# AjayGaneshC/medical-segmentation-pytorch

Hardware: AMD Instinct MI355X
Metric: images/sec (whole node) + val Dice, DUCKNet-17 352x352 at 1/2/4/8 MI355X (higher is better)
Workload: dtype bf16; 1 GPU; model=DUCKNet-17, global_batch=320, per_gpu_batch=320, seq_len=123904, step=SegTrainer.train_step, image_size=352, parallelism=dp1, impl=fused, optimizer=adam, loss=ce, syncbn=False, hipgraph=True

## Files before the change

csrc/bindings.cpp:

```cpp
#include <torch/extension.h>
#include <c10/hip/HIPStream.h>

#include <algorithm>
#include <vector>

#include "launchers.h"

namespace {

hipStream_t cur_stream() { return c10::hip::getCurrentHIPStream().stream(); }

#define CHECK_DEV(t) TORCH_CHECK((t).is_cuda() && (t).is_contiguous(), #t " must be a contiguous GPU tensor")
#define CHECK_BF16(t) CHECK_DEV(t); TORCH_CHECK((t).scalar_type() == at::kBFloat16, #t " must be bf16")
#define CHECK_F32(t) CHECK_DEV(t); TORCH_CHECK((t).scalar_type() == at::kFloat, #t " must be fp32")
#define CHECK_I64(t) CHECK_DEV(t); TORCH_CHECK((t).scalar_type() == at::kLong, #t " must be int64")

inline uint16_t* bf(const at::Tensor& t) { return reinterpret_cast<uint16_t*>(t.data_ptr()); }
inline float* f32(const at::Tensor& t) { return t.data_ptr<float>(); }
inline const float* f32_opt(const c10::optional<at::Tensor>& t) {
  if (!t.has_value() || !t->defined()) return nullptr;
  CHECK_F32(*t);
  return t->data_ptr<float>();
}
inline float* f32_opt_mut(const c10::optional<at::Tensor>& t) { return const_cast<float*>(f32_opt(t)); }
// ... 1602 lines not shown

extern "C" const char* msp_sources_sha();

PYBIND11_MODULE(_C, m) {
  m.doc() = "MI355X (gfx950) HIP kernels for medical_segmentation_pytorch_amd";
  m.def("conv_fwd", &conv_fwd, py::arg("xs"), py::arg("wp"), py::arg("ys"), py::arg("bias"), py::arg("stat_part"),
        py::arg("dims"), py::arg("dy"), py::arg("dx"), py::arg("trans"), py::arg("xc") = OptTensors{},
        py::arg("xrelu") = 0, py::arg("accumulate") = false, py::arg("gy") = OptTensors{},
        py::arg("gs") = OptTensors{}, py::arg("gk") = OptTensors{}, py::arg("grelu") = 0);
  m.def("conv_fwd_bn", &conv_fwd_bn, py::arg("xs"), py::arg("wp"), py::arg("ys"), py::arg("stat_part"), py::arg("dims"),
        py::arg("dy"), py::arg("dx"), py::arg("bn_y"), py::arg("bn_coef"), py::arg("relu"), py::arg("gy") = OptTensors{},
        py::arg("gs") = OptTensors{}, py::arg("gk") = OptTensors{}, py::arg("grelu") = 0);
  m.def("conv_wgrad", &conv_wgrad_t, py::arg("dys"), py::arg("xs"), py::arg("dw"), py::arg("dims"), py::arg("dy"),
        py::arg("dx"), py::arg("trans"), py::arg("xc") = OptTensors{}, py::arg("xrelu") = 0,
        py::arg("gy") = OptTensors{}, py::arg("gs") = OptTensors{}, py::arg("gk") = OptTensors{}, py::arg("grelu") = 0);
  m.def("conv_wgrad_uses_halo", &conv_wgrad_uses_halo_t);
  m.def("conv_pick_mi", &conv_pick_mi);
  m.def("conv_rows_alloc", &conv_rows_alloc);
  m.def("conv_stat_blocks", &conv_stat_blocks_t, py::arg("dims"), py::arg("dy"), py::arg("dx"), py::arg("trans") = false,
        py::arg("bwd") = false, py::arg("bne") = false);
  m.def("conv_uses_halo", &conv_uses_halo_t, py::arg("dims"), py::arg("dy"), py::arg("dx"), py::arg("trans"),
        py::arg("bwd") = false);
  m.def("conv_set_halo", [](bool on) { conv_set_halo(on ? 1 : 0); });
  m.def("conv_set_halo_split", [](int64_t mode) { conv_set_halo_split((int)mode); });
  m.def("conv_set_gemm", [](bool on) { conv_gemm_set(on ? 1 : 0); });
  m.def("conv_gemm_force_cfg", [](int64_t c) { conv_gemm_force_cfg((int)c); });
  m.def("conv_gemm_num_cfgs", []() { return conv_gemm_num_cfgs(); });
  m.def("conv_gemm_stamp_buffer", [](c10::optional<at::Tensor> buf) {
    if (!buf.has_value()) return conv_gemm_stamp_buffer(nullptr, 0);
    TORCH_CHECK(buf->is_cuda() && buf->is_contiguous() && buf->scalar_type() == at::kLong && buf->dim() == 2 &&
                    buf->size(1) == 4, "conv_gemm_stamp_buffer: a contiguous int64 [blocks][4] device tensor");
    return conv_gemm_stamp_buffer(buf->data_ptr(), buf->size(0));
  });
  m.def("conv_set_wgrad_gemm", [](int64_t mode) { conv_wgrad_gemm_set((int)mode); });
  m.def("conv_wgrad_gemm_force_cfg", [](int64_t c) { conv_wgrad_gemm_force_cfg((int)c); });
  m.def("conv_wgrad_gemm_num_cfgs", []() { return conv_wgrad_gemm_num_cfgs(); });
  m.def("conv_uses_wgrad_gemm", [](std::vector<int64_t> dims, std::vector<int64_t> dy, std::vector<int64_t> dx, bool trans) {
    return conv_wgrad_gemm_ok(make_geom(dims, dy, dx), trans);
  });
  m.def("conv_uses_gemm", [](std::vector<int64_t> dims, std::vector<int64_t> dy, std::vector<int64_t> dx, bool trans) {
    return conv_gemm_ok(make_geom(dims, dy, dx), trans);
  });
  m.def("conv_set_phase", [](bool on) { conv_set_phase(on ? 1 : 0); });
  m.def("pack_weight", &pack_weight_t);
  m.def("unpack_wgrad", &unpack_wgrad_t, py::arg("src"), py::arg("dst"), py::arg("nrow"), py::arg("nch"),
        py::arg("T"), py::arg("Cpk"), py::arg("Ktot"), py::arg("t_base"), py::arg("c_base"), py::arg("s_row"),
        py::arg("s_ch"), py::arg("accumulate"), py::arg("nrep") = 1, py::arg("rep_stride") = 0);
  m.def("conv_wgrad_replicas", &conv_wgrad_replicas_t, py::arg("dims"), py::arg("dy"), py::arg("dx"), py::arg("trans"),
        py::arg("bwd") = false, py::arg("pro") = false);
  m.def("pack_batch", &pack_batch_t);
  m.def("pack_per_block", &pack_per_block);
  m.def("bn_partial_blocks", [](int64_t P, int64_t Cp) { return bn_partial_blocks(P, Cp); });
  m.def("sum_stats", &sum_stats_t, py::arg("inputs"), py::arg("out"), py::arg("part"), py::arg("P"), py::arg("Cp"),
        py::arg("coefs") = OptTensors{}, py::arg("relu_mask") = 0);
  m.def("bn_reduce_partials", &bn_reduce_partials_t);
  m.def("bn_reduce_splits", [](int64_t nblk) { return bn_reduce_splits(nblk); });
  m.def("bn_collapse", &bn_collapse_t);
  m.def("bn_finalize", &bn_finalize_t);
  m.def("bn_reduce_finalize", &bn_reduce_finalize_t);
  m.def("bn_reduce_bwd_finalize", &bn_reduce_bwd_finalize_t);
  m.def("bn_rf_chunks", [](int64_t Cp) { return bn_rf_chunks((int)Cp); });
  m.def("bn_act_apply", &bn_act_apply_t);
  m.def("bn_act_apply_relu6", &bn_act_apply_relu6_t);
  m.def("bn_add_act", &bn_add_act_t);
  m.def("gconv_fwd", &gconv_fwd_t);
  m.def("relu6", &relu6_t);
// ... 158 lines not shown
```

csrc/conv_gemm.hip:

```cpp
#include <algorithm>

#include "common.h"
#include "launchers.h"

namespace {

typedef float f32x16_t __attribute__((ext_vector_type(16)));
typedef __attribute__((address_space(3))) void lds_void_t;

DEVI f32x16_t mfma32(const uint4& a, const uint4& b, f32x16_t c) {
#ifdef GK_KO_MFMA
  c[0] += __uint_as_float(a.x ^ b.y);
  return c;
#else
  return __builtin_amdgcn_mfma_f32_32x32x16_bf16(as_bf16x8(a), as_bf16x8(b), c, 0, 0, 0);
#endif
}

DEVI void st_stream8(uint16_t* p, uint32_t lo, uint32_t hi) {
#ifdef GK_KO_STORE
  if (lo == 0x7fc17fc1u && hi == 0x12345678u) *reinterpret_cast<uint2*>(p) = make_uint2(lo, hi);
#else
  *reinterpret_cast<uint2*>(p) = make_uint2(lo, hi);
#endif
}

__device__ __attribute__((aligned(64))) uint4 g_zero_page[4];

DEVI void glds16(const void* src, uint32_t lds) {
#ifdef GK_KO_DMA
  return;
#endif
  unsigned keep;
  asm volatile("s_mov_b32 %0, m0\n\ts_mov_b32 m0, %2\n\ts_nop 0\n\tglobal_load_lds_dwordx4 %1, off\n\ts_mov_b32 m0, %0"
               : "=&s"(keep) : "v"(src), "s"(lds) : "memory");
}

typedef __attribute__((address_space(3))) uint8_t lds_u8_t;

#ifdef GK_STAMP
DEVI unsigned long long gk_clock() {
  unsigned long long t;
  __builtin_amdgcn_sched_barrier(0);
  asm volatile("s_memrealtime %0\n\ts_waitcnt lgkmcnt(0)" : "=s"(t)::"memory");
  __builtin_amdgcn_sched_barrier(0);
  return t;
}
#endif


struct KPos { int t, gi, cl; };

DEVI KPos kpos_init(int k, int Cgi, int Gi) {
  const int Cip = Gi * Cgi;
  KPos p;
  p.t = k / Cip;
  const int rem = k - p.t * Cip;
  p.gi = rem / Cgi;
  p.cl = rem - p.gi * Cgi;
  return p;
}

DEVI void kpos_advance(KPos& p, int by, int Cgi, int Gi) {
  p.cl += by;
  while (p.cl >= Cgi) {
    p.cl -= Cgi;
    if (++p.gi == Gi) { p.gi = 0; ++p.t; }
  }
}

struct GemmGeom {
  long M, OHW;
  int n_co, nk;
  int ps, py, px, OWp;
  long OHWp, OW, OHWf;
  long apitch;
#ifdef GK_STAMP
  unsigned long long* stamp;
  long stamp_cap;
#endif
};

template <int WM, int WN, int FM, int FN, int NS, int BK>
struct GemmCfg {
  static constexpr int NW = WM * WN, NT = 64 * NW;
  static constexpr int TCO = 32 * WM * FM, TPX = 32 * WN * FN;
  static constexpr int ROWB = BK * 2, SLOTS = BK / 8, RPI = 1024 / ROWB;
  static constexpr int A_BYTES = TCO * ROWB, B_BYTES = TPX * ROWB, STAGE = A_BYTES + B_BYTES;
  static constexpr int A_INS = TCO / RPI / NW, B_INS = TPX / RPI / NW;
  static constexpr int LDS = NS * STAGE;
  static_assert(BK == 64 || BK == 32, "stage width");
  static_assert(TCO % (RPI * NW) == 0 && TPX % (RPI * NW) == 0, "tile rows must split evenly over the waves");
  static_assert(2 * WN * TCO * 4 <= NS * STAGE, "stats scratch must fit in the staging LDS");
  static_assert(NS >= 2 && NS <= 5 && (NS - 2) * (A_INS + B_INS) < 64, "pipeline depth / vmcnt range");
  static_assert(NW % 2 == 0, "one logical k slot per lane across the wave's DMA instructions");
  static DEVI int swz(int row) { return BK == 64 ? ((row >> 1) & 7) : ((row >> 2) & 3); }
};

struct TapGrid {
  int kw, y0, ys, x0, xs;
  int akw, ar0, ars, ac0, acs;
};

template <int WM, int WN, int FM, int FN, int NS, int BK, bool BNE, int OCC = 2>
__global__ __launch_bounds__(64 * WM * WN, OCC) void conv_gemm_kernel(ConvArgs a, GemmGeom gg, TapGrid tg) {
  using C = GemmCfg<WM, WN, FM, FN, NS, BK>;
  constexpr int kRowB = C::ROWB, RPI = C::RPI;
  const ConvGeom& g = a.g;
  extern __shared__ __attribute__((aligned(16))) uint8_t smem[];

  const int tid = threadIdx.x, lane = tid & 63, wave = __builtin_amdgcn_readfirstlane(tid >> 6);
  const uint32_t sbase = (uint32_t)(uintptr_t)(lds_u8_t*)smem;
#ifdef GK_STAMP
  const unsigned long long ts0 = gk_clock();
  unsigned long long ts1 = ts0;
#endif

  const int nwg = gridDim.x, orig = blockIdx.x;
  const int xq = nwg / 8, xr = nwg % 8, xcd = orig % 8;
  const int wgid = (xcd < xr ? xcd * (xq + 1) : xr * (xq + 1) + (xcd - xr) * xq) + orig / 8;
  const int co_t = wgid % gg.n_co;
  const long px_t = wgid / gg.n_co;
  const int co0 = co_t * C::TCO;
  const long px0 = px_t * C::TPX;
  const int rows = g.Go * g.Cgo;
  const int Cgi = g.Cgi, Gi = g.Gi;
  const int IHW = g.IH * g.IW;

  const int ls = (lane % C::SLOTS) ^ C::swz(RPI * wave + lane / C::SLOTS);
  const uint16_t* zero = reinterpret_cast<const uint16_t*>(g_zero_page);
  const uint16_t* a_src[C::A_INS];
#pragma unroll
  for (int j = 0; j < C::A_INS; ++j) {
    const int co = co0 + RPI * (j * C::NW + wave) + lane / C::SLOTS;
    a_src[j] = a.w + (long)(co < rows ? co : 0) * gg.apitch + 8 * ls;
#ifdef GK_KO_AMISS
    a_src[j] = a.w + 8 * ls;
#endif
  }
  long b_pix[C::B_INS];
  uint32_t b_vm[C::B_INS];
#pragma unroll
  for (int j = 0; j < C::B_INS; ++j) {
    const long m = px0 + RPI * (j * C::NW + wave) + lane / C::SLOTS;
    b_pix[j] = 0;
    b_vm[j] = 0u;
    if (m < gg.M) {
      const int n = (int)(m / gg.OHW);
      const int r = (int)(m - (long)n * gg.OHW);
      const int oh = r / g.OW, ow = r - (r / g.OW) * g.OW;
      const int ih0 = oh * g.stride, iw0 = ow * g.stride;
      b_pix[j] = ((long)n * IHW + (long)ih0 * g.IW + iw0) * Cgi;
#ifdef GK_KO_BMISS
      b_pix[j] = ((long)(ih0 % 4) * g.IW + (iw0 % 8)) * Cgi;
#endif
      uint32_t vm = 0u;
      int tr = 0, tc = 0;
      for (int t = 0; t < g.T; ++t) {
        const int ih = ih0 + tg.y0 + tr * tg.ys, iw = iw0 + tg.x0 + tc * tg.xs;
        if ((unsigned)ih < (unsigned)g.IH && (unsigned)iw < (unsigned)g.IW) vm |= 1u << t;
// ... 12 lines not shown
    g0 = rem / Cgi;
    cl0 = rem - g0 * Cgi;
    tr0 = t0 / tg.kw;
    tc0 = t0 - tr0 * tg.kw;
    toff0 = ((long)(tg.y0 + tr0 * tg.ys) * g.IW + (tg.x0 + tc0 * tg.xs)) * Cgi;
  };
  walk_to(0);
  auto gptr = [&](int q) {
    const uint16_t* xb = a.x[0];
#pragma unroll
    for (int u = 1; u < kMaxGroups; ++u) xb = q == u ? a.x[u] : xb;
    return xb;
  };
  const uint16_t* xg0 = gptr(g0);
  const uint16_t* xg1 = gptr(g0 + 1 == Gi ? 0 : g0 + 1);

  const int Cip_ = Gi * Cgi;
  auto stage = [&](int kt, uint32_t sb) {
    const int kb = kt * BK;
    int g1 = g0 + 1, t1 = t0, tr1 = tr0, tc1 = tc0;
    long toff1 = toff0;
    if (g1 == Gi) {
      g1 = 0;
      ++t1;
      toff1 += dcol;
      if (++tc1 == tg.kw) { tc1 = 0; ++tr1; toff1 += drow; }
    }
    const int rem0 = Cgi - cl0;
    const bool nx = 8 * ls >= rem0;
    const int dA0 = ((tg.ar0 + tr0 * tg.ars) * tg.akw + tg.ac0 + tc0 * tg.acs - t0) * Cip_;
    const int dA1 = t1 < g.T ? ((tg.ar0 + tr1 * tg.ars) * tg.akw + tg.ac0 + tc1 * tg.acs - t1) * Cip_ : dA0;
    const int ka = kb + (nx ? dA1 : dA0);
#pragma unroll
    for (int j = 0; j < C::A_INS; ++j) glds16(a_src[j] + ka, sb + (RPI * (j * C::NW + wave)) * kRowB);
    const int t = nx ? t1 : t0;
#ifdef GK_OLD_XSEL
    const uint16_t* base = (nx ? gptr(g1) : gptr(g0)) + (nx ? toff1 + (8 * ls - rem0) : toff0 + (cl0 + 8 * ls));
#else
    asm volatile("" : "+s"(xg0), "+s"(xg1));
    const uint16_t* base = (nx ? xg1 : xg0) + (nx ? toff1 + (8 * ls - rem0) : toff0 + (cl0 + 8 * ls));
#endif
    const bool tin = t < 32;
#pragma unroll
    for (int j = 0; j < C::B_INS; ++j) {
      const bool ok = tin && ((b_vm[j] >> t) & 1u);
      glds16(ok ? (const void*)(base + b_pix[j]) : (const void*)zero,
             sb + C::A_BYTES + (RPI * (j * C::NW + wave)) * kRowB);
    }
    cl0 += BK;
    if (cl0 >= Cgi) {
      cl0 -= Cgi; g0 = g1; t0 = t1; tr0 = tr1; tc0 = tc1; toff0 = toff1;
      xg0 = xg1;
      xg1 = gptr(g0 + 1 == Gi ? 0 : g0 + 1);
    }
  };

  const int wm = wave / WN, wn = wave - (wave / WN) * WN;
  const int lr = lane & 31, lh = lane >> 5;
  const int key = C::swz(lr);
  constexpr int KS = BK / 16;
  int soff[KS];
#pragma unroll
  for (int s = 0; s < KS; ++s) soff[s] = (((2 * s + lh) ^ key) << 4);
  const int a_row0 = (wm * FM * 32 + lr) * kRowB;
  const int b_row0 = C::A_BYTES + (wn * FN * 32 + lr) * kRowB;

  f32x16_t acc[FM][FN];
#pragma unroll
  for (int i = 0; i < FM; ++i)
#pragma unroll
    for (int j = 0; j < FN; ++j)
#pragma unroll
      for (int e = 0; e < 16; ++e) acc[i][j][e] = 0.f;

  constexpr int INS = C::A_INS + C::B_INS;
  const int nk = gg.nk;
#pragma unroll
  for (int p = 0; p < NS - 1; ++p)
    if (p < nk) stage(p, sbase + p * C::STAGE);
  for (int kt = 0; kt < nk; ++kt) {
    const int ahead = min(nk - 1 - kt, NS - 2);
    if (NS >= 5 && ahead >= 3) asm volatile("s_waitcnt vmcnt(%0)" ::"n"(3 * INS) : "memory");
    else if (NS >= 4 && ahead >= 2) asm volatile("s_waitcnt vmcnt(%0)" ::"n"(2 * INS) : "memory");
    else if (ahead >= 1) asm volatile("s_waitcnt vmcnt(%0)" ::"n"(INS) : "memory");
    else asm volatile("s_waitcnt vmcnt(0)" ::: "memory");
    __builtin_amdgcn_s_barrier();
    __builtin_amdgcn_sched_barrier(0);
    if (kt + NS - 1 < nk) stage(kt + NS - 1, sbase + ((kt + NS - 1) % NS) * C::STAGE);
    const uint8_t* cur = smem + (kt % NS) * C::STAGE;
#ifdef GK_STAMP
    if (kt == 0) ts1 = gk_clock();
#endif
#pragma unroll
    for (int s = 0; s < KS; ++s) {
      uint4 af[FM], bfr[FN];
#pragma unroll
#ifdef GK_KO_LDS
      for (int i = 0; i < FM; ++i) af[i] = make_uint4(kt + i, s, lane, 0);
#pragma unroll
      for (int j = 0; j < FN; ++j) bfr[j] = make_uint4(kt, j + s, 0, lane);
#else
      for (int i = 0; i < FM; ++i) af[i] = *reinterpret_cast<const uint4*>(cur + a_row0 + i * 32 * kRowB + soff[s]);
#pragma unroll
      for (int j = 0; j < FN; ++j) bfr[j] = *reinterpret_cast<const uint4*>(cur + b_row0 + j * 32 * kRowB + soff[s]);
#endif
#pragma unroll
      for (int i = 0; i < FM; ++i)
#pragma unroll
        for (int j = 0; j < FN; ++j) acc[i][j] = mfma32(af[i], bfr[j], acc[i][j]);
    }
  }
  __syncthreads();
#ifdef GK_STAMP
  const unsigned long long ts2 = gk_clock();
#endif

  float* s_st = reinterpret_cast<float*>(smem);
  const bool stats = a.stat_part != nullptr;
#pragma unroll
  for (int i = 0; i < FM; ++i) {
    const int rb = wm * FM * 32 + i * 32;
    uint16_t* yb[4];
    int cl4[4];
    float cs[16], cq[16];
#pragma unroll
    for (int q = 0; q < 4; ++q) {
      const int cb = co0 + rb + 8 * q + 4 * lh;
      const int og = cb < rows ? cb / g.Cgo : 0;
      cl4[q] = cb - og * g.Cgo;
      uint16_t* yg = a.y[0];
#pragma unroll
      for (int t = 1; t < kMaxGroups; ++t) yg = og == t ? a.y[t] : yg;
      yb[q] = cb < rows ? yg + cl4[q] : nullptr;
    }
#pragma unroll
    for (int e = 0; e < 16; ++e) { cs[e] = 0.f; cq[e] = 0.f; }
#pragma unroll
    for (int j = 0; j < FN; ++j) {
      long m = px0 + wn * FN * 32 + j * 32 + lr;
      if (m >= gg.M) continue;
      if (gg.ps) {
        const long n = m / gg.OHWp, r = m - n * gg.OHWp;
        const long oh = r / gg.OWp, ow = r - oh * gg.OWp;
        m = n * gg.OHWf + (gg.py + gg.ps * oh) * gg.OW + gg.px + gg.ps * ow;
      }
#pragma unroll
      for (int q = 0; q < 4; ++q) {
        if (yb[q] == nullptr) continue;
        uint16_t* yp = yb[q] + m * g.Cgo;
        float v[4];
#pragma unroll
        for (int r = 0; r < 4; ++r) v[r] = acc[i][j][4 * q + r];
        if (a.bias != nullptr) {
#pragma unroll
          for (int r = 0; r < 4; ++r) v[r] = cl4[q] + r < g.Cgo_l ? v[r] + a.bias[cl4[q] + r] : 0.f;
        }
        if (!BNE && a.accum) {
          const uint2 ov = *reinterpret_cast<const uint2*>(yp);
          v[0] += __uint_as_float(ov.x << 16); v[1] += __uint_as_float(ov.x & 0xffff0000u);
          v[2] += __uint_as_float(ov.y << 16); v[3] += __uint_as_float(ov.y & 0xffff0000u);
        }
        const uint32_t lo = pack2(v[0], v[1]), hi = pack2(v[2], v[3]);
        st_stream8(yp, lo, hi);
        const float w4[4] = {__uint_as_float(lo << 16), __uint_as_float(lo & 0xffff0000u),
                             __uint_as_float(hi << 16), __uint_as_float(hi & 0xffff0000u)};
        if constexpr (BNE) {
          const int cb = cl4[q];
          const uint2 yy = *reinterpret_cast<const uint2*>(a.bn_y + m * g.Cgo + cb);
          const float4 sc = *reinterpret_cast<const float4*>(a.bn_coef + cb);
          const float4 sh = *reinterpret_cast<const float4*>(a.bn_coef + g.Cgo + cb);
          const float4 mu = *reinterpret_cast<const float4*>(a.bn_coef + 2 * g.Cgo + cb);
          const float y4[4] = {__uint_as_float(yy.x << 16), __uint_as_float(yy.x & 0xffff0000u),
                               __uint_as_float(yy.y << 16), __uint_as_float(yy.y & 0xffff0000u)};
          const float s4[4] = {sc.x, sc.y, sc.z, sc.w}, h4[4] = {sh.x, sh.y, sh.z, sh.w};
          const float m4[4] = {mu.x, mu.y, mu.z, mu.w};
#pragma unroll
          for (int r = 0; r < 4; ++r) {
            const float gr = (!a.bn_relu || fmaf(y4[r], s4[r], h4[r]) > 0.f) ? w4[r] : 0.f;
            cs[4 * q + r] += gr;
            cq[4 * q + r] = fmaf(gr, y4[r] - m4[r], cq[4 * q + r]);
          }
        } else {
#pragma unroll
          for (int r = 0; r < 4; ++r) {
            cs[4 * q + r] += w4[r];
            cq[4 * q + r] = fmaf(w4[r], w4[r], cq[4 * q + r]);
          }
        }
      }
    }
    if (stats) {
#pragma unroll
      for (int e = 0; e < 16; ++e) {
        float s = row16_sum(cs[e]), q = row16_sum(cq[e]);
        s += __shfl_xor(s, 16, 64);
        q += __shfl_xor(q, 16, 64);
        if (lr == 0) {
          const int row = rb + 8 * (e >> 2) + 4 * lh + (e & 3);
          s_st[(wn * 2 + 0) * C::TCO + row] = s;
          s_st[(wn * 2 + 1) * C::TCO + row] = q;
        }
      }
    }
  }
  if (stats) {
    __syncthreads();
    constexpr int HALVES = C::TPX / 128, WPH = WN / HALVES;
    static_assert(C::TPX % 128 == 0 && WN % HALVES == 0, "128-pixel stat rows");
    const long nrow = (gg.M + 127) / 128;
    for (int e = tid; e < HALVES * C::TCO; e += C::NT) {
      const int hb = e / C::TCO, c = e - hb * C::TCO;
      const int co = co0 + c;
      const long srow = px0 / 128 + hb;
      if (co >= rows || srow >= nrow) continue;
      float s = 0.f, q = 0.f;
#pragma unroll
      for (int w = 0; w < WPH; ++w) {
        const int wv = hb * WPH + w;
        s += s_st[(wv * 2 + 0) * C::TCO + c];
        q += s_st[(wv * 2 + 1) * C::TCO + c];
      }
      a.stat_part[(srow * 2 + 0) * rows + co] = s;
      a.stat_part[(srow * 2 + 1) * rows + co] = q;
    }
  }
#ifdef GK_STAMP
  const unsigned long long ts3 = gk_clock();
  if (tid == 0 && gg.stamp != nullptr && wgid < gg.stamp_cap) {
    unsigned long long* sp = gg.stamp + 4 * (long)wgid;
    sp[0] = ts0; sp[1] = ts1; sp[2] = ts2; sp[3] = ts3;
  }
#endif
}

struct CfgId { int wm, wn, fm, fn, ns, bk; };
constexpr CfgId kCfgs[] = {
    {2, 2, 3, 2, 2, 64},
    {2, 2, 2, 2, 2, 64},
    {1, 4, 3, 1, 2, 64},
    {1, 4, 5, 1, 2, 64},
    {2, 2, 1, 2, 2, 64},
    {2, 2, 2, 2, 4, 32},
    {2, 2, 3, 2, 4, 32},
    {2, 2, 4, 2, 3, 32},
    {2, 2, 2, 2, 5, 32},
    {2, 2, 2, 2, 2, 32},
};
constexpr int kNumCfgs = sizeof(kCfgs) / sizeof(kCfgs[0]);
constexpr int kPlannerCfgs = 5;
constexpr int kOccCfg = 9;
constexpr int kGemmTPX = 128;

int g_gemm_mode = -1;
int g_gemm_cfg = -1;

void gemm_env() {
  if (g_gemm_mode < 0) {
    const char* e = getenv("MSP_CONV_GEMM");
    g_gemm_mode = (e == nullptr || e[0] != '0') ? 1 : 0;
  }
}

int gemm_pick_cfg(int rows, int nk64) {
  if (g_gemm_cfg >= 0) return g_gemm_cfg;
  int best = 0;
  double best_cost = 1e30;
  for (int c = 0; c < kPlannerCfgs; ++c) {
    const int tco = 32 * kCfgs[c].wm * kCfgs[c].fm;
    const int tiles = cdiv(rows, tco);
    const double cost = (double)tiles * (tco + 48.0);
    if (cost < best_cost - 1e-9) { best_cost = cost; best = c; }
  }
  const int tb = 32 * kCfgs[best].wm * kCfgs[best].fm, to = 32 * kCfgs[kOccCfg].wm * kCfgs[kOccCfg].fm;
  if (nk64 <= 12 && (double)cdiv(rows, to) * to <= 1.35 * cdiv(rows, tb) * tb) return kOccCfg;
  return best;
}

bool tap_grid(const ConvGeom& g, TapGrid& tg) {
  for (int kw = 1; kw <= g.T; ++kw) {
    if (g.T % kw != 0) continue;
    const int kh = g.T / kw;
    tg.kw = kw; tg.y0 = g.dy[0]; tg.x0 = g.dx[0];
    tg.ys = kh > 1 ? g.dy[kw] - g.dy[0] : 0;
    tg.xs = kw > 1 ? g.dx[1] - g.dx[0] : 0;
    bool ok = true;
    for (int t = 0; t < g.T && ok; ++t)
      ok = g.dy[t] == tg.y0 + (t / kw) * tg.ys && g.dx[t] == tg.x0 + (t % kw) * tg.xs;
    if (ok) return true;
  }
  return false;
}

struct GemmPhase {
  int ps = 0, py = 0, px = 0, OHf = 0, OWf = 0;
  long apitch = 0;
  int akw = 0, ar0 = 0, ars = 1, ac0 = 0, acs = 1;
};

#ifdef GK_STAMP
unsigned long long* g_stamp = nullptr;
long g_stamp_cap = 0;
#endif

template <int WM, int WN, int FM, int FN, int NS, int BK, bool BNE, int OCC = 2>
void launch_gemm(const ConvArgs& a, const GemmPhase& ph, hipStream_t s) {
  using C = GemmCfg<WM, WN, FM, FN, NS, BK>;
  const ConvGeom& g = a.g;
  GemmGeom gg;
  gg.OHW = (long)g.OH * g.OW;
  gg.M = (long)g.N * gg.OHW;
  gg.n_co = cdiv(g.Go * g.Cgo, C::TCO);
  gg.nk = cdiv(g.Kp, BK);
  gg.ps = ph.ps; gg.py = ph.py; gg.px = ph.px; gg.OWp = g.OW;
  gg.OHWp = gg.OHW; gg.OW = ph.OWf; gg.OHWf = (long)ph.OHf * ph.OWf;
  gg.apitch = ph.apitch > 0 ? ph.apitch : g.Kp;
  const long blocks = (long)cdiv(gg.M, C::TPX) * gg.n_co;
#ifdef GK_STAMP
  gg.stamp = g_stamp; gg.stamp_cap = g_stamp_cap;
#endif
  static bool attr = false;
  if (!attr) {
    (void)hipFuncSetAttribute(reinterpret_cast<const void*>(&conv_gemm_kernel<WM, WN, FM, FN, NS, BK, BNE, OCC>),
                              hipFuncAttributeMaxDynamicSharedMemorySize, C::LDS);
    attr = true;
  }
  TapGrid tg;
  (void)tap_grid(g, tg);
  if (ph.akw > 0) {
    tg.akw = ph.akw; tg.ar0 = ph.ar0; tg.ars = ph.ars; tg.ac0 = ph.ac0; tg.acs = ph.acs;
  } else {
    tg.akw = tg.kw; tg.ar0 = 0; tg.ars = 1; tg.ac0 = 0; tg.acs = 1;
  }
  hipLaunchKernelGGL((conv_gemm_kernel<WM, WN, FM, FN, NS, BK, BNE, OCC>), dim3((unsigned)blocks), dim3(C::NT), C::LDS, s, a, gg,
                     tg);
}

template <bool BNE>
int dispatch_gemm(const ConvArgs& a, int cfg, const GemmPhase& ph, hipStream_t s) {
  switch (cfg) {
    case 0: launch_gemm<2, 2, 3, 2, 2, 64, BNE>(a, ph, s); return 0;
    case 1: launch_gemm<2, 2, 2, 2, 2, 64, BNE>(a, ph, s); return 0;
    case 2: launch_gemm<1, 4, 3, 1, 2, 64, BNE>(a, ph, s); return 0;
    case 3: launch_gemm<1, 4, 5, 1, 2, 64, BNE>(a, ph, s); return 0;
    case 4: launch_gemm<2, 2, 1, 2, 2, 64, BNE>(a, ph, s); return 0;
    case 5: launch_gemm<2, 2, 2, 2, 4, 32, BNE>(a, ph, s); return 0;
    case 6: launch_gemm<2, 2, 3, 2, 4, 32, BNE>(a, ph, s); return 0;
    case 7: launch_gemm<2, 2, 4, 2, 3, 32, BNE>(a, ph, s); return 0;
    case 8: launch_gemm<2, 2, 2, 2, 5, 32, BNE>(a, ph, s); return 0;
    case 9: launch_gemm<2, 2, 2, 2, 2, 32, BNE, 4>(a, ph, s); return 0;
  }
  return 1;
}

}

static bool gemm_geom_ok(const ConvGeom& g, int min_c) {
  if (g.Cgi < min_c || g.Cgi % 8 != 0 || g.T > 30) return false;
  TapGrid tg;
  if (!tap_grid(g, tg)) return false;
  const long M = (long)g.N * g.OH * g.OW;
  return M >= 1 && (long)cdiv(M, kGemmTPX) * cdiv(g.Go * g.Cgo, 64) < (1L << 31);
}

bool conv_gemm_ok(const ConvGeom& g, bool trans) {
  gemm_env();
  if (!g_gemm_mode || trans) return false;
  return gemm_geom_ok(g, g.stride > 1 ? 32 : 64);
}

static int gemm_tile_for(const ConvGeom& g) {
  const int cfg = gemm_pick_cfg(g.Go * g.Cgo, cdiv(g.Kp, 64));
  return (g.Cgi < 64 && kCfgs[cfg].bk == 64) ? kOccCfg : cfg;
}

void conv_gemm_set(int on) { gemm_env(); g_gemm_mode = on ? 1 : 0; }
void conv_gemm_force_cfg(int cfg) { gemm_env(); g_gemm_cfg = (cfg >= 0 && cfg < kNumCfgs) ? cfg : -1; }
int conv_gemm_num_cfgs() { return kNumCfgs; }
int conv_gemm_stamp_buffer(void* buf, long cap) {
#ifdef GK_STAMP
  g_stamp = static_cast<unsigned long long*>(buf);
  g_stamp_cap = buf != nullptr ? cap : 0;
  return 1;
#else
  (void)buf; (void)cap;
  return 0;
#endif
}

long conv_gemm_stat_blocks(const ConvGeom& g) { return cdiv((long)g.N * g.OH * g.OW, kGemmTPX); }

int conv_gemm(const ConvArgs& a, hipStream_t s) {
  gemm_env();
  for (int i = 0; i < a.g.Gi; ++i)
    if (a.xc[i] != nullptr) return 2;
  const int cfg = gemm_tile_for(a.g);
  const GemmPhase ph;
  return a.bn_y != nullptr ? dispatch_gemm<true>(a, cfg, ph, s) : dispatch_gemm<false>(a, cfg, ph, s);
}

int conv_gemm_phase(const ConvArgs& a0, const int* tA, int KW, int s_, int py, int px, int OHf, int OWf,
                    hipStream_t s) {
  gemm_env();
  ConvArgs a = a0;
  ConvGeom& g = a.g;
  const long apitch = g.Kp;
  g.Kp = (g.T * g.Gi * g.Cgi + 31) / 32 * 32;
  if (g.T < 1 || !g_gemm_mode || !gemm_geom_ok(g, 32) || a.bn_y != nullptr || a.stat_part != nullptr) return 1;
  for (int i = 0; i < g.Gi; ++i)
    if (a.xc[i] != nullptr || a.gy[i] != nullptr) return 1;
  TapGrid tg;
  if (!tap_grid(g, tg)) return 1;
  GemmPhase ph;
  ph.ps = s_; ph.py = py; ph.px = px; ph.OHf = OHf; ph.OWf = OWf; ph.apitch = apitch;
  const int kh = g.T / tg.kw;
  ph.akw = KW;
  ph.ar0 = tA[0] / KW; ph.ac0 = tA[0] % KW;
  ph.ars = kh > 1 ? tA[tg.kw] / KW - ph.ar0 : 0;
  ph.acs = tg.kw > 1 ? tA[1] % KW - ph.ac0 : 0;
  for (int v = 0; v < g.T; ++v)
    if (tA[v] != (ph.ar0 + (v / tg.kw) * ph.ars) * KW + ph.ac0 + (v % tg.kw) * ph.acs) return 1;
  const int cfg = gemm_tile_for(g);
  return dispatch_gemm<false>(a, cfg, ph, s) == 0 ? 0 : 2;
}
```

csrc/conv_wgrad_gemm.hip:

```cpp
#include <algorithm>

#include "common.h"
#include "launchers.h"

namespace {

typedef float f32x16_t __attribute__((ext_vector_type(16)));
typedef short s16x4_t __attribute__((ext_vector_type(4)));
typedef __attribute__((address_space(3))) uint8_t lds_u8_t;

DEVI f32x16_t mfma32(const uint4& a, const uint4& b, f32x16_t c) {
#ifdef GK_KO_MFMA
  c[0] += __uint_as_float(a.x ^ b.y);
  return c;
#else
  return __builtin_amdgcn_mfma_f32_32x32x16_bf16(as_bf16x8(a), as_bf16x8(b), c, 0, 0, 0);
#endif
}

__device__ __attribute__((aligned(64))) uint4 g_wg_zero_page[4];

DEVI void glds16(const void* src, uint32_t lds) {
#ifdef GK_KO_DMA
  return;
// ... 263 lines not shown
    g_wg_mode = e == nullptr ? 1 : (e[0] == '0' ? 0 : (e[0] == '2' ? 2 : 1));
  }
}

int wg_pick(int rows, int KT, bool pro) {
  if (g_wg_cfg >= 0 && (!pro || wg_pro_ok(kWgCfgs[g_wg_cfg].wn, kWgCfgs[g_wg_cfg].fn))) return g_wg_cfg;
  int best = 0;
  double best_cost = 1e30;
  for (int c = 0; c < kNumWgCfgs; ++c) {
    if (pro && !wg_pro_ok(kWgCfgs[c].wn, kWgCfgs[c].fn)) continue;
    const int tco = 32 * kWgCfgs[c].wm * kWgCfgs[c].fm, tk = 32 * kWgCfgs[c].wn * kWgCfgs[c].fn;
    const double nt = (double)cdiv(rows, tco) * cdiv(KT, tk);
    const double cost = nt * ((double)tco * tk + g_wg_stage_cost * (tco + tk));
    if (cost < best_cost) { best_cost = cost; best = c; }
  }
  return best;
}

bool wg_tap_grid(const ConvGeom& g, WgGeom& w) {
  for (int kw = 1; kw <= g.T; ++kw) {
    if (g.T % kw != 0) continue;
    const int kh = g.T / kw;
    w.kw = kw; w.ty0 = g.dy[0]; w.tx0 = g.dx[0];
    w.tys = kh > 1 ? g.dy[kw] - g.dy[0] : 0;
    w.txs = kw > 1 ? g.dx[1] - g.dx[0] : 0;
    bool ok = true;
    for (int t = 0; t < g.T && ok; ++t) ok = g.dy[t] == w.ty0 + (t / kw) * w.tys && g.dx[t] == w.tx0 + (t % kw) * w.txs;
    if (ok) return true;
  }
  return false;
}

struct WgPlan { int cfg; WgGeom w; long blocks; int nsplit; };

WgPlan wg_plan(const ConvGeom& g, bool pro) {
  WgPlan p{};
  p.cfg = wg_pick(g.Go * g.Cgo, g.T * g.Gi * g.Cgi, pro);
  const WgCfg& c = kWgCfgs[p.cfg];
  WgGeom& w = p.w;
  (void)wg_tap_grid(g, w);
  w.M = (long)g.N * g.OH * g.OW;
  w.KT = g.T * g.Gi * g.Cgi;
  w.n_co = cdiv(g.Go * g.Cgo, 32 * c.wm * c.fm);
  w.n_k = cdiv(w.KT, 32 * c.wn * c.fn);
  w.nstages = (int)((w.M + kBP - 1) / kBP);
  const long ntile = (long)w.n_co * w.n_k;
  const long target = c.wm * c.wn >= 8 ? g_wg_blocks / 2 : g_wg_blocks;
  long ns = std::max(1L, std::min((long)w.nstages, target / std::max(1L, ntile)));
  w.stages_per_split = (int)((w.nstages + ns - 1) / ns);
  ns = (w.nstages + w.stages_per_split - 1) / w.stages_per_split;
  p.nsplit = (int)ns;
  p.blocks = ns * ntile;
  w.d_ohw = make_fastdiv((uint32_t)(g.OH * g.OW));
  w.d_ow = make_fastdiv((uint32_t)g.OW);
  return p;
}

template <int WM, int WN, int FM, int FN>
int launch_wg(const WgradPtrs& P, float* dw, const ConvGeom& g, const WgPlan& p, bool pro, hipStream_t s) {
  constexpr int LDS = 2 * kBP * (32 * WM * FM + 32 * WN * FN) * 2;
  static bool attr[2] = {false, false};
  if (pro) {
    if constexpr (!wg_pro_ok(WN, FN)) {
      return 1;
    } else {
    if (!attr[1]) {
      (void)hipFuncSetAttribute(reinterpret_cast<const void*>(&conv_wgrad_gemm_kernel<WM, WN, FM, FN, true>),
                                hipFuncAttributeMaxDynamicSharedMemorySize, LDS);
      attr[1] = true;
    }
    hipLaunchKernelGGL((conv_wgrad_gemm_kernel<WM, WN, FM, FN, true>), dim3((unsigned)p.blocks), dim3(64 * WM * WN),
                       LDS, s, P, dw, g, p.w);
    return 0;
    }
  }
  if (!attr[0]) {
    (void)hipFuncSetAttribute(reinterpret_cast<const void*>(&conv_wgrad_gemm_kernel<WM, WN, FM, FN, false>),
                              hipFuncAttributeMaxDynamicSharedMemorySize, LDS);
    attr[0] = true;
  }
  hipLaunchKernelGGL((conv_wgrad_gemm_kernel<WM, WN, FM, FN, false>), dim3((unsigned)p.blocks), dim3(64 * WM * WN), LDS,
                     s, P, dw, g, p.w);
  return 0;
}


}

bool conv_wgrad_gemm_ok(const ConvGeom& g, bool trans) {
  wg_env();
  if (!g_wg_mode || trans || g.Cgi % 8 != 0 || g.Cgo % 8 != 0) return false;
  WgGeom w{};
  if (!wg_tap_grid(g, w)) return false;
  const long M = (long)g.N * g.OH * g.OW;
  return M < (1L << 31) - 2 * kBP;
}

int conv_wgrad_gemm_replicas(const ConvGeom& g, bool pro) {
  wg_env();
  return wg_plan(g, pro).nsplit;
}

void conv_wgrad_gemm_set(int mode) { wg_env(); g_wg_mode = mode < 0 ? 0 : (mode > 2 ? 2 : mode); }
int conv_wgrad_gemm_mode() { wg_env(); return g_wg_mode; }
void conv_wgrad_gemm_force_cfg(int cfg) { wg_env(); g_wg_cfg = (cfg >= 0 && cfg < kNumWgCfgs) ? cfg : -1; }
int conv_wgrad_gemm_num_cfgs() { return kNumWgCfgs; }

int conv_wgrad_gemm(const WgradPtrs& P, float* dw, const ConvGeom& g, bool prologue, hipStream_t s) {
  const WgPlan p = wg_plan(g, prologue);
  switch (p.cfg) {
    case 0: return launch_wg<2, 2, 2, 2>(P, dw, g, p, prologue, s);
    case 1: return launch_wg<1, 4, 1, 1>(P, dw, g, p, prologue, s);
    case 2: return launch_wg<2, 2, 1, 2>(P, dw, g, p, prologue, s);
    case 3: return launch_wg<2, 2, 2, 1>(P, dw, g, p, prologue, s);
    case 4: return launch_wg<1, 4, 2, 1>(P, dw, g, p, prologue, s);
    case 5: return launch_wg<2, 2, 4, 1>(P, dw, g, p, prologue, s);
    case 6: return launch_wg<2, 4, 4, 2>(P, dw, g, p, prologue, s);
    case 7: return launch_wg<2, 4, 2, 2>(P, dw, g, p, prologue, s);
    case 8: return launch_wg<4, 2, 2, 2>(P, dw, g, p, prologue, s);
  }
  return 1;
}
```

csrc/launchers.h:

```cpp
#pragma once
#include <hip/hip_runtime.h>
#include <stdint.h>

constexpr int kMaxTaps = 49;

constexpr int kMaxGroups = 8;
struct ConvGeom {
  int N, IH, IW;
  int Gi, Cgi;
  int OH, OW;
  int Go, Cgo, Cgo_l;
  int T, Kp;
  int stride;
  int dy[kMaxTaps], dx[kMaxTaps];
};

struct ConvArgs {
  const uint16_t* x[kMaxGroups];
  uint16_t* y[kMaxGroups];
  const uint16_t* w;
  const float* bias;
  float* stat_part;
  const uint16_t* bn_y;
  const float* bn_coef;
// ... 17 lines not shown
  const float* gs[kMaxGroups];
  const float* gk[kMaxGroups];
  unsigned grelu;
};

bool conv_wgrad_gemm_ok(const ConvGeom& g, bool trans);
int conv_wgrad_gemm_replicas(const ConvGeom& g, bool pro = false);
int conv_wgrad_gemm(const WgradPtrs& P, float* dw, const ConvGeom& g, bool prologue, hipStream_t s);
void conv_wgrad_gemm_set(int mode);
int conv_wgrad_gemm_mode();
void conv_wgrad_gemm_force_cfg(int cfg);
int conv_wgrad_gemm_num_cfgs();

int conv_pick_mi(int rows);
int conv_rows_alloc(int rows);
void conv_set_halo(int on);
void conv_set_halo_split(int mode);
void conv_set_phase(int on);
bool conv_uses_halo(const ConvGeom& g, bool trans, bool bwd = false);
long conv_stat_blocks(const ConvGeom& g, bool trans = false, bool bwd = false, bool bne = false);
bool conv_wgrad_uses_halo(const ConvGeom& g, bool trans);
int conv_igemm(const ConvArgs& a, bool trans, hipStream_t s);
const char* conv_error_string(int rc);

bool conv_gemm_ok(const ConvGeom& g, bool trans);
long conv_gemm_stat_blocks(const ConvGeom& g);
int conv_gemm(const ConvArgs& a, hipStream_t s);
int conv_gemm_phase(const ConvArgs& a, const int* tA, int KW, int s_, int py, int px, int OHf, int OWf,
                    hipStream_t s);
void conv_gemm_set(int on);
void conv_gemm_force_cfg(int cfg);
int conv_gemm_num_cfgs();
int conv_gemm_stamp_buffer(void* buf, long cap);
int conv_plan_selfcheck(int verbose);
int conv_wgrad_replicas(const ConvGeom& g, bool trans, bool bwd = false, bool pro = false);
int conv_wgrad(const uint16_t* const* dy, const uint16_t* const* x, float* dw, const ConvGeom& g, bool trans,
               const float* const* xc, unsigned xrelu, hipStream_t s, const uint16_t* const* gy = nullptr,
               const float* const* gs = nullptr, const float* const* gk = nullptr, unsigned grelu = 0);
void pack_weight(const float* src, uint16_t* dst, int nrow, int nch, int T, int Cpk, int Kp, int t_base,
                 int c_base, long s_row, long s_ch, hipStream_t s);
void pack_batch(const int64_t* jobs, const int* prefix, int njobs, int total_blocks, hipStream_t s);
int pack_per_block();
void unpack_wgrad(const float* src, float* dst, int nrow, int nch, int T, int Cpk, int Ktot, int t_base, int c_base,
                  long s_row, long s_ch, bool accumulate, int nrep, long rep_stride, hipStream_t s);

constexpr int kMaxSumInputs = 8;
constexpr int kTailMax = 6;
constexpr int kTailMaxCp = 512;
long bn_partial_blocks(long P, int Cp);
long bn_tail_blocks(long P, int Cp);
void bn_tail_partial(const uint16_t* dz, const uint16_t* ys, const float* ostats, const float* ocoef, int orelu, int k,
                     const uint16_t* const* y, const float* const* st, unsigned relu, float* part, long P, int Cp,
                     hipStream_t s);
void bn_tail_apply(const uint16_t* dz, const uint16_t* ys, const float* ostats, const float* ocoef, int orelu, int k,
                   const uint16_t* const* y, const float* const* st, const float* const* coef, unsigned relu,
                   uint16_t* const* dy, long P, int Cp, hipStream_t s, uint16_t* g = nullptr);
void sum_stats(const uint16_t* const* inputs, const float* const* coefs, unsigned relu_mask, int k, uint16_t* out,
               float* part, long P, int Cp, hipStream_t s);
int bn_reduce_splits(long nblk);
void bn_reduce_partials(const float* part, long nblk, int width, int col_off, int Cp, double* tmp, hipStream_t s);
void bn_collapse(const double* tmp, int S, int Cp, double* out, hipStream_t s);
void bn_finalize(const double* tmp, int S, int C, int Cp, float count, const float* gamma, const float* beta,
                 float* running_mean, float* running_var, float momentum, float eps, int training,
                 float* scale, float* shift, float* mean, float* invstd, hipStream_t s);
int bn_rf_chunks(int Cp);
void bn_reduce_finalize(const float* part, long nblk, int width, int col_off, int C, int Cp, double* tmp,
// ... 282 lines not shown
```

Measured before the change: 674.0 images/sec.

## Add wide-pixel and non-power-of-two channel tiles to conv GEMM planner

Adds four new forward conv GEMM tile configurations with 160/96/128/192 output-channel and 128/256 pixel tiles. A planner cost model picks them by comparing staged bytes per pixel and wave-quantization round-up against the existing 128-pixel choice. To support channel tiles that do not split evenly across waves, weight DMA is predicated per wave and vmcnt waits become per-wave counts. BN statistics reduction is regrouped for 256-pixel tiles. The goal is less redundant staging of A/B tiles and less tile padding on wide layers, at the cost of more kernel instantiations, more complex waits and a heuristic that may misselect. Also adds plan-logging counters exposed to Python.

```diff
diff --git a/csrc/bindings.cpp b/csrc/bindings.cpp
--- a/csrc/bindings.cpp
+++ b/csrc/bindings.cpp
@@ -1658,6 +1658,13 @@
                     buf->size(1) == 4, "conv_gemm_stamp_buffer: a contiguous int64 [blocks][4] device tensor");
     return conv_gemm_stamp_buffer(buf->data_ptr(), buf->size(0));
   });
+  auto plan_log_list = [](const ConvPlanLog& l) {
+    return std::vector<int64_t>{l.launches, l.blocks, l.staged, l.staged_full, l.cfg, l.tco, l.tpx, l.bk, l.ns, l.nk};
+  };
+  m.def("conv_gemm_plan_log", [plan_log_list](bool reset) { return plan_log_list(conv_gemm_plan_log(reset)); },
+        py::arg("reset") = true);
+  m.def("conv_wgrad_gemm_plan_log",
+        [plan_log_list](bool reset) { return plan_log_list(conv_wgrad_gemm_plan_log(reset)); }, py::arg("reset") = true);
   m.def("conv_set_wgrad_gemm", [](int64_t mode) { conv_wgrad_gemm_set((int)mode); });
   m.def("conv_wgrad_gemm_force_cfg", [](int64_t c) { conv_wgrad_gemm_force_cfg((int)c); });
   m.def("conv_wgrad_gemm_num_cfgs", []() { return conv_wgrad_gemm_num_cfgs(); });
diff --git a/csrc/conv_gemm.hip b/csrc/conv_gemm.hip
--- a/csrc/conv_gemm.hip
+++ b/csrc/conv_gemm.hip
@@ -1,4 +1,5 @@
 #include <algorithm>
+#include <cmath>
 
 #include "common.h"
 #include "launchers.h"
@@ -48,6 +49,19 @@
 }
 #endif
 
+
+template <int N>
+DEVI void wait_vm() { asm volatile("s_waitcnt vmcnt(%0)" ::"n"(N) : "memory"); }
+template <int LVL, int B, int A>
+DEVI void wait_stages(int na) {
+  static_assert(LVL * (A + B) < 64, "vmcnt range");
+  if constexpr (A == 0) {
+    wait_vm<LVL * B>();
+  } else {
+    if (na == A) wait_vm<LVL * (A + B)>();
+    else wait_stages<LVL, B, A - 1>(na);
+  }
+}
 
 struct KPos { int t, gi, cl; };
 
@@ -75,6 +89,7 @@
   int ps, py, px, OWp;
   long OHWp, OW, OHWf;
   long apitch;
+  int sg;
 #ifdef GK_STAMP
   unsigned long long* stamp;
   long stamp_cap;
@@ -87,11 +102,13 @@
   static constexpr int TCO = 32 * WM * FM, TPX = 32 * WN * FN;
   static constexpr int ROWB = BK * 2, SLOTS = BK / 8, RPI = 1024 / ROWB;
   static constexpr int A_BYTES = TCO * ROWB, B_BYTES = TPX * ROWB, STAGE = A_BYTES + B_BYTES;
-  static constexpr int A_INS = TCO / RPI / NW, B_INS = TPX / RPI / NW;
+  static constexpr int A_TOT = TCO / RPI, A_INS = (A_TOT + NW - 1) / NW, B_INS = TPX / RPI / NW;
   static constexpr int LDS = NS * STAGE;
   static_assert(BK == 64 || BK == 32, "stage width");
-  static_assert(TCO % (RPI * NW) == 0 && TPX % (RPI * NW) == 0, "tile rows must split evenly over the waves");
-  static_assert(2 * WN * TCO * 4 <= NS * STAGE, "stats scratch must fit in the staging LDS");
+  static_assert(TCO % RPI == 0 && TPX % (RPI * NW) == 0, "pixel rows must split evenly over the waves");
+  static constexpr int STAT_SLOTS = TPX > 128 ? TPX / 32 : WN;
+  static_assert(2 * STAT_SLOTS * TCO * 4 <= NS * STAGE, "stats scratch must fit in the staging LDS");
+  static_assert(TPX == 128 || (TPX == 256 && FN % 2 == 0), "stat groups of 1 or 2 fragments inside a wave");
   static_assert(NS >= 2 && NS <= 5 && (NS - 2) * (A_INS + B_INS) < 64, "pipeline depth / vmcnt range");
   static_assert(NW % 2 == 0, "one logical k slot per lane across the wave's DMA instructions");
   static DEVI int swz(int row) { return BK == 64 ? ((row >> 1) & 7) : ((row >> 2) & 3); }
@@ -126,6 +143,9 @@
   const int rows = g.Go * g.Cgo;
   const int Cgi = g.Cgi, Gi = g.Gi;
   const int IHW = g.IH * g.IW;
+
+  const int a_real = (min(C::TCO, rows - co0) + RPI - 1) / RPI;
+  const int na = wave < a_real ? (a_real - wave + C::NW - 1) / C::NW : 0;
 
   const int ls = (lane % C::SLOTS) ^ C::swz(RPI * wave + lane / C::SLOTS);
   const uint16_t* zero = reinterpret_cast<const uint16_t*>(g_zero_page);
@@ -204,7 +224,8 @@
     const int dA1 = t1 < g.T ? ((tg.ar0 + tr1 * tg.ars) * tg.akw + tg.ac0 + tc1 * tg.acs - t1) * Cip_ : dA0;
     const int ka = kb + (nx ? dA1 : dA0);
 #pragma unroll
-    for (int j = 0; j < C::A_INS; ++j) glds16(a_src[j] + ka, sb + (RPI * (j * C::NW + wave)) * kRowB);
+    for (int j = 0; j < C::A_INS; ++j)
+      if (j < na) glds16(a_src[j] + ka, sb + (RPI * (j * C::NW + wave)) * kRowB);
     const int t = nx ? t1 : t0;
 #ifdef GK_OLD_XSEL
     const uint16_t* base = (nx ? gptr(g1) : gptr(g0)) + (nx ? toff1 + (8 * ls - rem0) : toff0 + (cl0 + 8 * ls));
@@ -245,17 +266,19 @@
 #pragma unroll
       for (int e = 0; e < 16; ++e) acc[i][j][e] = 0.f;
 
-  constexpr int INS = C::A_INS + C::B_INS;
   const int nk = gg.nk;
 #pragma unroll
   for (int p = 0; p < NS - 1; ++p)
     if (p < nk) stage(p, sbase + p * C::STAGE);
   for (int kt = 0; kt < nk; ++kt) {
     const int ahead = min(nk - 1 - kt, NS - 2);
-    if (NS >= 5 && ahead >= 3) asm volatile("s_waitcnt vmcnt(%0)" ::"n"(3 * INS) : "memory");
-    else if (NS >= 4 && ahead >= 2) asm volatile("s_waitcnt vmcnt(%0)" ::"n"(2 * INS) : "memory");
-    else if (ahead >= 1) asm volatile("s_waitcnt vmcnt(%0)" ::"n"(INS) : "memory");
-    else asm volatile("s_waitcnt vmcnt(0)" ::: "memory");
+    bool waited = false;
+    if constexpr (NS >= 5)
+      if (ahead >= 3) { wait_stages<3, C::B_INS, C::A_INS>(na); waited = true; }
+    if constexpr (NS >= 4)
+      if (!waited && ahead >= 2) { wait_stages<2, C::B_INS, C::A_INS>(na); waited = true; }
+    if (!waited && ahead >= 1) { wait_stages<1, C::B_INS, C::A_INS>(na); waited = true; }
+    if (!waited) wait_vm<0>();
     __builtin_amdgcn_s_barrier();
     __builtin_amdgcn_sched_barrier(0);
     if (kt + NS - 1 < nk) stage(kt + NS - 1, sbase + ((kt + NS - 1) % NS) * C::STAGE);
@@ -289,6 +312,8 @@
 
   float* s_st = reinterpret_cast<float*>(smem);
   const bool stats = a.stat_part != nullptr;
+  constexpr bool WIDE = C::TPX > 128;
+  const int sg = WIDE ? gg.sg : FN;
 #pragma unroll
   for (int i = 0; i < FM; ++i) {
     const int rb = wm * FM * 32 + i * 32;
@@ -305,12 +330,31 @@
       for (int t = 1; t < kMaxGroups; ++t) yg = og == t ? a.y[t] : yg;
       yb[q] = cb < rows ? yg + cl4[q] : nullptr;
     }
+    auto reduce_to = [&](int slot) {
+#pragma unroll
+      for (int e = 0; e < 16; ++e) {
+        float s = row16_sum(cs[e]), q = row16_sum(cq[e]);
+        s += __shfl_xor(s, 16, 64);
+        q += __shfl_xor(q, 16, 64);
+        if (lr == 0) {
+          const int row = rb + 8 * (e >> 2) + 4 * lh + (e & 3);
+          s_st[(slot * 2 + 0) * C::TCO + row] = s;
+          s_st[(slot * 2 + 1) * C::TCO + row] = q;
+        }
+      }
+    };
 #pragma unroll
     for (int e = 0; e < 16; ++e) { cs[e] = 0.f; cq[e] = 0.f; }
 #pragma unroll
     for (int j = 0; j < FN; ++j) {
+      if constexpr (WIDE) {
+        if (j > 0 && j % sg == 0) {
+#pragma unroll
+          for (int e = 0; e < 16; ++e) { cs[e] = 0.f; cq[e] = 0.f; }
+        }
+      }
       long m = px0 + wn * FN * 32 + j * 32 + lr;
-      if (m >= gg.M) continue;
+      if (m < gg.M) {
       if (gg.ps) {
         const long n = m / gg.OHWp, r = m - n * gg.OHWp;
         const long oh = r / gg.OWp, ow = r - oh * gg.OWp;
@@ -360,25 +404,20 @@
           }
         }
       }
-    }
-    if (stats) {
-#pragma unroll
-      for (int e = 0; e < 16; ++e) {
-        float s = row16_sum(cs[e]), q = row16_sum(cq[e]);
-        s += __shfl_xor(s, 16, 64);
-        q += __shfl_xor(q, 16, 64);
-        if (lr == 0) {
-          const int row = rb + 8 * (e >> 2) + 4 * lh + (e & 3);
-          s_st[(wn * 2 + 0) * C::TCO + row] = s;
-          s_st[(wn * 2 + 1) * C::TCO + row] = q;
-        }
       }
+      if constexpr (WIDE) {
+        if (stats && j % sg == sg - 1) reduce_to((wn * FN + j) / sg);
+      }
+    }
+    if constexpr (!WIDE) {
+      if (stats) reduce_to(wn);
     }
   }
   if (stats) {
     __syncthreads();
-    constexpr int HALVES = C::TPX / 128, WPH = WN / HALVES;
-    static_assert(C::TPX % 128 == 0 && WN % HALVES == 0, "128-pixel stat rows");
+    constexpr int HALVES = C::TPX / 128;
+    static_assert(C::TPX % 128 == 0, "128-pixel stat rows");
+    const int WPH = WIDE ? 4 / sg : WN;
     const long nrow = (gg.M + 127) / 128;
     for (int e = tid; e < HALVES * C::TCO; e += C::NT) {
       const int hb = e / C::TCO, c = e - hb * C::TCO;
@@ -386,7 +425,6 @@
       const long srow = px0 / 128 + hb;
       if (co >= rows || srow >= nrow) continue;
       float s = 0.f, q = 0.f;
-#pragma unroll
       for (int w = 0; w < WPH; ++w) {
         const int wv = hb * WPH + w;
         s += s_st[(wv * 2 + 0) * C::TCO + c];
@@ -417,10 +455,18 @@
     {2, 2, 4, 2, 3, 32},
     {2, 2, 2, 2, 5, 32},
     {2, 2, 2, 2, 2, 32},
+    {1, 4, 5, 2, 2, 32},
+    {1, 4, 3, 2, 2, 32},
+    {2, 2, 2, 4, 2, 32},
+    {2, 4, 3, 2, 2, 64},
 };
 constexpr int kNumCfgs = sizeof(kCfgs) / sizeof(kCfgs[0]);
 constexpr int kPlannerCfgs = 5;
 constexpr int kOccCfg = 9;
+constexpr int kWide160 = 10, kWide96 = 11, kWide128 = 12, kWide192 = 13;
+constexpr int kCfgBlocksPerCU[] = {2, 2, 2, 2, 2, 2, 2, 2, 2, 4, 2, 3, 2, 1};
+static_assert(sizeof(kCfgBlocksPerCU) / sizeof(int) == kNumCfgs, "one entry per configuration");
+constexpr int kPlanCUs = 256;
 constexpr int kGemmTPX = 128;
 
 int g_gemm_mode = -1;
@@ -433,8 +479,7 @@
   }
 }
 
-int gemm_pick_cfg(int rows, int nk64) {
-  if (g_gemm_cfg >= 0) return g_gemm_cfg;
+int gemm_pick_cfg128(int rows, int nk64) {
   int best = 0;
   double best_cost = 1e30;
   for (int c = 0; c < kPlannerCfgs; ++c) {
@@ -446,6 +491,38 @@
   const int tb = 32 * kCfgs[best].wm * kCfgs[best].fm, to = 32 * kCfgs[kOccCfg].wm * kCfgs[kOccCfg].fm;
   if (nk64 <= 12 && (double)cdiv(rows, to) * to <= 1.35 * cdiv(rows, tb) * tb) return kOccCfg;
   return best;
+}
+
+double gemm_staged_per_px(int rows, int c) {
+  const int tco = 32 * kCfgs[c].wm * kCfgs[c].fm, tpx = 32 * kCfgs[c].wn * kCfgs[c].fn;
+  return (double)cdiv(rows, tco) * (tco + tpx) / tpx;
+}
+double gemm_rounds(int rows, long M, int c) {
+  const int tco = 32 * kCfgs[c].wm * kCfgs[c].fm, tpx = 32 * kCfgs[c].wn * kCfgs[c].fn;
+  return (double)cdiv(M, (long)tpx) * cdiv(rows, tco) / (kPlanCUs * kCfgBlocksPerCU[c]);
+}
+double gemm_round_up(int rows, long M, int c) {
+  const double x = gemm_rounds(rows, M, c);
+  return x <= 2.0 ? std::ceil(x) / x : 1.0;
+}
+
+int gemm_pick_cfg(int rows, int nk64, int gi, int cgi, long M, bool phase) {
+  if (g_gemm_cfg >= 0) return g_gemm_cfg;
+  const int c128 = gemm_pick_cfg128(rows, nk64);
+  if (gi != 1 || cgi < 64 || phase) return c128;
+  if (c128 == kOccCfg) {
+    const int w = rows <= 96 ? kWide96 : kWide128;
+    const bool ok = nk64 >= 8 && gemm_rounds(rows, M, w) >= 1.0 && gemm_round_up(rows, M, w) <= gemm_round_up(rows, M, c128);
+    return ok ? w : c128;
+  }
+  const double cost128 = gemm_staged_per_px(rows, c128) * gemm_round_up(rows, M, c128);
+  if (gemm_rounds(rows, M, kWide160) >= 1.0 &&
+      gemm_staged_per_px(rows, kWide160) * gemm_round_up(rows, M, kWide160) <= 0.78 * cost128)
+    return kWide160;
+  if (nk64 >= 64 && gemm_rounds(rows, M, kWide192) >= 1.0 &&
+      gemm_staged_per_px(rows, kWide192) * gemm_round_up(rows, M, kWide192) <= 0.72 * cost128)
+    return kWide192;
+  return c128;
 }
 
 bool tap_grid(const ConvGeom& g, TapGrid& tg) {
@@ -468,6 +545,8 @@
   long apitch = 0;
   int akw = 0, ar0 = 0, ars = 1, ac0 = 0, acs = 1;
 };
+
+ConvPlanLog g_plan_log{};
 
 #ifdef GK_STAMP
 unsigned long long* g_stamp = nullptr;
@@ -486,7 +565,21 @@
   gg.ps = ph.ps; gg.py = ph.py; gg.px = ph.px; gg.OWp = g.OW;
   gg.OHWp = gg.OHW; gg.OW = ph.OWf; gg.OHWf = (long)ph.OHf * ph.OWf;
   gg.apitch = ph.apitch > 0 ? ph.apitch : g.Kp;
+  {
+    const int c128 = gemm_pick_cfg128(g.Go * g.Cgo, cdiv(g.Kp, 64));
+    gg.sg = kCfgs[(g.Cgi < 64 && kCfgs[c128].bk == 64) ? kOccCfg : c128].fn;
+  }
   const long blocks = (long)cdiv(gg.M, C::TPX) * gg.n_co;
+  {
+    const int rows = g.Go * g.Cgo;
+    const long a_rows = (long)(gg.n_co - 1) * C::TCO + cdiv(rows - (gg.n_co - 1) * C::TCO, C::RPI) * C::RPI;
+    const long px_tiles = cdiv(gg.M, C::TPX);
+    g_plan_log.launches += 1;
+    g_plan_log.blocks += blocks;
+    g_plan_log.staged += px_tiles * gg.nk * (a_rows + (long)gg.n_co * C::TPX) * C::ROWB;
+    g_plan_log.staged_full += blocks * gg.nk * C::STAGE;
+    g_plan_log.tco = C::TCO; g_plan_log.tpx = C::TPX; g_plan_log.bk = BK; g_plan_log.ns = NS; g_plan_log.nk = gg.nk;
+  }
 #ifdef GK_STAMP
   gg.stamp = g_stamp; gg.stamp_cap = g_stamp_cap;
 #endif
@@ -520,6 +613,10 @@
     case 7: launch_gemm<2, 2, 4, 2, 3, 32, BNE>(a, ph, s); return 0;
     case 8: launch_gemm<2, 2, 2, 2, 5, 32, BNE>(a, ph, s); return 0;
     case 9: launch_gemm<2, 2, 2, 2, 2, 32, BNE, 4>(a, ph, s); return 0;
+    case 10: launch_gemm<1, 4, 5, 2, 2, 32, BNE>(a, ph, s); return 0;
+    case 11: launch_gemm<1, 4, 3, 2, 2, 32, BNE, 3>(a, ph, s); return 0;
+    case 12: launch_gemm<2, 2, 2, 4, 2, 32, BNE>(a, ph, s); return 0;
+    case 13: launch_gemm<2, 4, 3, 2, 2, 64, BNE>(a, ph, s); return 0;
   }
   return 1;
 }
@@ -540,14 +637,19 @@
   return gemm_geom_ok(g, g.stride > 1 ? 32 : 64);
 }
 
-static int gemm_tile_for(const ConvGeom& g) {
-  const int cfg = gemm_pick_cfg(g.Go * g.Cgo, cdiv(g.Kp, 64));
+static int gemm_tile_for(const ConvGeom& g, bool phase = false) {
+  const int cfg = gemm_pick_cfg(g.Go * g.Cgo, cdiv(g.Kp, 64), g.Gi, g.Cgi, (long)g.N * g.OH * g.OW, phase);
   return (g.Cgi < 64 && kCfgs[cfg].bk == 64) ? kOccCfg : cfg;
 }
 
 void conv_gemm_set(int on) { gemm_env(); g_gemm_mode = on ? 1 : 0; }
 void conv_gemm_force_cfg(int cfg) { gemm_env(); g_gemm_cfg = (cfg >= 0 && cfg < kNumCfgs) ? cfg : -1; }
 int conv_gemm_num_cfgs() { return kNumCfgs; }
+ConvPlanLog conv_gemm_plan_log(bool reset) {
+  const ConvPlanLog l = g_plan_log;
+  if (reset) g_plan_log = ConvPlanLog{};
+  return l;
+}
 int conv_gemm_stamp_buffer(void* buf, long cap) {
 #ifdef GK_STAMP
   g_stamp = static_cast<unsigned long long*>(buf);
@@ -566,6 +668,7 @@
   for (int i = 0; i < a.g.Gi; ++i)
     if (a.xc[i] != nullptr) return 2;
   const int cfg = gemm_tile_for(a.g);
+  g_plan_log.cfg = cfg;
   const GemmPhase ph;
   return a.bn_y != nullptr ? dispatch_gemm<true>(a, cfg, ph, s) : dispatch_gemm<false>(a, cfg, ph, s);
 }
@@ -591,6 +694,7 @@
   ph.acs = tg.kw > 1 ? tA[1] % KW - ph.ac0 : 0;
   for (int v = 0; v < g.T; ++v)
     if (tA[v] != (ph.ar0 + (v / tg.kw) * ph.ars) * KW + ph.ac0 + (v % tg.kw) * ph.acs) return 1;
-  const int cfg = gemm_tile_for(g);
+  const int cfg = gemm_tile_for(g, true);
+  g_plan_log.cfg = cfg;
   return dispatch_gemm<false>(a, cfg, ph, s) == 0 ? 0 : 2;
 }
diff --git a/csrc/conv_wgrad_gemm.hip b/csrc/conv_wgrad_gemm.hip
--- a/csrc/conv_wgrad_gemm.hip
+++ b/csrc/conv_wgrad_gemm.hip
@@ -319,6 +319,7 @@
 }
 
 struct WgPlan { int cfg; WgGeom w; long blocks; int nsplit; };
+ConvPlanLog g_wg_plan_log{};
 
 WgPlan wg_plan(const ConvGeom& g, bool pro) {
   WgPlan p{};
@@ -346,6 +347,15 @@
 template <int WM, int WN, int FM, int FN>
 int launch_wg(const WgradPtrs& P, float* dw, const ConvGeom& g, const WgPlan& p, bool pro, hipStream_t s) {
   constexpr int LDS = 2 * kBP * (32 * WM * FM + 32 * WN * FN) * 2;
+  {
+    const long stages = (long)p.w.n_co * p.w.n_k * p.w.nstages;
+    g_wg_plan_log.launches += 1;
+    g_wg_plan_log.blocks += p.blocks;
+    g_wg_plan_log.staged += stages * (LDS / 2);
+    g_wg_plan_log.staged_full += stages * (LDS / 2);
+    g_wg_plan_log.cfg = p.cfg; g_wg_plan_log.tco = 32 * WM * FM; g_wg_plan_log.tpx = 32 * WN * FN;
+    g_wg_plan_log.bk = kBP; g_wg_plan_log.ns = 2; g_wg_plan_log.nk = p.w.stages_per_split;
+  }
   static bool attr[2] = {false, false};
   if (pro) {
     if constexpr (!wg_pro_ok(WN, FN)) {
@@ -392,6 +402,11 @@
 int conv_wgrad_gemm_mode() { wg_env(); return g_wg_mode; }
 void conv_wgrad_gemm_force_cfg(int cfg) { wg_env(); g_wg_cfg = (cfg >= 0 && cfg < kNumWgCfgs) ? cfg : -1; }
 int conv_wgrad_gemm_num_cfgs() { return kNumWgCfgs; }
+ConvPlanLog conv_wgrad_gemm_plan_log(bool reset) {
+  const ConvPlanLog l = g_wg_plan_log;
+  if (reset) g_wg_plan_log = ConvPlanLog{};
+  return l;
+}
 
 int conv_wgrad_gemm(const WgradPtrs& P, float* dw, const ConvGeom& g, bool prologue, hipStream_t s) {
   const WgPlan p = wg_plan(g, prologue);
diff --git a/csrc/launchers.h b/csrc/launchers.h
--- a/csrc/launchers.h
+++ b/csrc/launchers.h
@@ -73,6 +73,9 @@
 void conv_gemm_force_cfg(int cfg);
 int conv_gemm_num_cfgs();
 int conv_gemm_stamp_buffer(void* buf, long cap);
+struct ConvPlanLog { long launches, blocks, staged, staged_full; int cfg, tco, tpx, bk, ns, nk; };
+ConvPlanLog conv_gemm_plan_log(bool reset);
+ConvPlanLog conv_wgrad_gemm_plan_log(bool reset);
 int conv_plan_selfcheck(int verbose);
 int conv_wgrad_replicas(const ConvGeom& g, bool trans, bool bwd = false, bool pro = false);
 int conv_wgrad(const uint16_t* const* dy, const uint16_t* const* x, float* dw, const ConvGeom& g, bool trans,
```

Result: no change. 676.1 images/sec (median of 4 runs) (+0.3%).
